# thiery-lab/manifold-mcmc-for-diffusions

Hardware: AMD Instinct MI355X
Metric: constrained-leapfrog steps/sec (all chains), FHN noisy-obs 400 sub-steps (higher is better)
Workload: dtype f64; 1 GPU; FHN noisy-obs, T=100 obs, S=400 steps/obs, R=5 obs/subseq, sigma_y=0.1, 256 chains per GPU (BASELINE.json configs[1]), Newton solver, standard splitting; chains_per_gpu=256, global_chains=256, dim_q=80106, traj_len=16, stepping=chmc_leapfrog_steps per trajectory (batched steps), chain_steps_nominal=152576, parallelism=chains x1 (no data-path collective, 1 gather), ranks_joined=1, collective_world_size=1, collective_route=torch.distributed gather, overlap_halves=-1

## Files before the change

### manifold_mcmc_for_diffusions_amd/context.py

```python
import ctypes as C
import numpy as np
from . import _lib
from ._lib import ChmcConfig, as_c, ptr, iptr, check

MODEL_IDS = {"fhn": 0, "sir": 1, "fhn_nb": 2}
STATUS_NAMES = {0: "ok", 1: "not_converged", 2: "diverged", 3: "non_reversible", -1: "inactive"}


class ChmcContext:
    def __init__(self, model, obs_interval, num_steps_per_obs, num_obs_per_subseq, y_seq, sigma=None,
                 use_gaussian_splitting=False, num_chains=1, device=0):
        L = _lib.lib()
        self.L = L
        y = as_c(np.asarray(y_seq).reshape(-1))
        self._y = y
        cfg = ChmcConfig(
            model=MODEL_IDS[model] if isinstance(model, str) else int(model), num_obs=len(y),
            num_steps_per_obs=int(num_steps_per_obs),
            num_obs_per_subseq=0 if num_obs_per_subseq is None else int(num_obs_per_subseq),
            noisy=2 if isinstance(sigma, str) else int(sigma is not None),
            use_gaussian_splitting=int(bool(use_gaussian_splitting)),
            num_chains=int(num_chains), device=int(device), obs_interval=float(obs_interval),
            sigma=0.0 if sigma is None or isinstance(sigma, str) else float(sigma), y_seq=ptr(y))
        h = C.c_void_p()
# ... 296 lines not shown
                      divergence_tol=1e10, max_iters=50, reverse_check_tol=2e-8):
        dt = as_c(np.broadcast_to(np.asarray(dt, dtype=np.float64), (self.B,)))
        act = None if active is None else np.ascontiguousarray(active, dtype=np.int32)
        status = np.zeros(self.B, dtype=np.int32)
        itf, itb = np.zeros(self.B, dtype=np.int32), np.zeros(self.B, dtype=np.int32)
        rev = np.zeros(self.B)
        check(self.L.chmc_leapfrog_step(self.h, ptr(dt), iptr(act), int(n_inner_step), int(newton), constraint_tol,
                                        position_tol, divergence_tol, int(max_iters), reverse_check_tol, iptr(status),
                                        iptr(itf), iptr(itb), ptr(rev)), "chmc_leapfrog_step")
        return dict(status=status, iters_fwd=itf, iters_bwd=itb, rev_err=rev)

    def leapfrog_steps(self, dt, n_steps, active=None, n_inner_step=1, newton=True, constraint_tol=1e-9, position_tol=1e-8,
                       divergence_tol=1e10, max_iters=50, reverse_check_tol=2e-8):
        dt = as_c(np.broadcast_to(np.asarray(dt, dtype=np.float64), (self.B,)))
        act = None if active is None else np.ascontiguousarray(active, dtype=np.int32)
        per_chain = None if np.isscalar(n_steps) else np.ascontiguousarray(np.broadcast_to(n_steps, (self.B,)), dtype=np.int32)
        n_all = int(n_steps) if per_chain is None else 0
        ndone, status = np.zeros(self.B, dtype=np.int32), np.zeros(self.B, dtype=np.int32)
        itf, itb = np.zeros(self.B, dtype=np.int32), np.zeros(self.B, dtype=np.int32)
        rev = np.zeros(self.B)
        check(self.L.chmc_leapfrog_steps(self.h, ptr(dt), iptr(act), iptr(per_chain), n_all, int(n_inner_step), int(newton),
                                         constraint_tol, position_tol, divergence_tol, int(max_iters), reverse_check_tol,
                                         iptr(ndone), iptr(status), iptr(itf), iptr(itb), ptr(rev)), "chmc_leapfrog_steps")
        return dict(n_done=ndone, status=status, iters_fwd=itf, iters_bwd=itb, rev_err=rev)

    def comm_init(self, id128, rank, world):
        buf = (C.c_char * 128).from_buffer_copy(bytes(id128))
        check(self.L.chmc_comm_init(self.h, buf, int(rank), int(world)), "chmc_comm_init")
        self.comm_world = int(world)

    @staticmethod
    def comm_unique_id():
        buf = (C.c_char * 128)()
        check(_lib.lib().chmc_comm_unique_id(buf), "chmc_comm_unique_id")
        return bytes(buf)

    def gather_samples_device(self, local_dev_ptr, count, gathered_dev_ptr):
        check(self.L.chmc_gather_samples(self.h, C.c_void_p(local_dev_ptr), int(count), C.c_void_p(gathered_dev_ptr)),
              "chmc_gather_samples")

    def comm_info(self):
        wd, rk = C.c_int(0), C.c_int(0)
        check(self.L.chmc_comm_info(self.h, C.byref(wd), C.byref(rk)), "chmc_comm_info")
        return wd.value, rk.value

    def comm_destroy(self):
        check(self.L.chmc_comm_destroy(self.h), "chmc_comm_destroy")

    def diagnostics(self):
        out = (C.c_longlong * 80)()
        check(self.L.chmc_get_diagnostics(self.h, out), "chmc_get_diagnostics")
        v = np.array(out[:], dtype=np.int64)
        return dict(par_scan=v[:64], gram_mfma_launches=int(v[64]), gram_valu_launches=int(v[65]),
                    retract_kernel_launches=int(v[66]), traj_kernel_launches=int(v[67]), extra=v[68:80])

    def counters(self):
        out = (C.c_longlong * 8)()
        check(self.L.chmc_get_counters(self.h, out), "chmc_get_counters")
        keys = ("constr", "jacob_constr_blocks", "lu_jacob_product_blocks", "chol_gram_blocks",
                "grad_log_det_sqrt_gram", "leapfrog_step", "projection_iterations", "_")
        return dict(zip(keys, (int(v) for v in out)))
```

### manifold_mcmc_for_diffusions_amd/csrc/backend_hip.h

```cpp
#pragma once
#include <hip/hip_runtime.h>

static thread_local hipStream_t g_stream = nullptr;
static thread_local hipStream_t g_streams[3] = {nullptr, nullptr, nullptr};
static thread_local int g_device = -1;
static hipError_t g_first_err = hipSuccess;

static inline void note(hipError_t e) {
  if (e != hipSuccess && g_first_err == hipSuccess) g_first_err = e;
}
static int dev_set(int device) {
  hipError_t e = hipSetDevice(device);
  if (e != hipSuccess) {
    g_err = std::string("hipSetDevice: ") + hipGetErrorString(e);
    return -1;
  }
  return 0;
}
static int dev_init(int device) {
  int n = 0;
  hipError_t e = hipGetDeviceCount(&n);
  if (e != hipSuccess || n <= 0) {
    g_err = std::string("no HIP device available (") + hipGetErrorString(e) + ")";
    return -1;
// ... 61 lines not shown
  __syncthreads();
  if (threadIdx.x == 0) {
    const unsigned t = atomicAdd(ticket, 1u);
    if (t == gridDim.x - 1) {
      const int v = atomicAdd(counter, 0);
      *ticket = 0u;
      __hip_atomic_store(host_out, v, __ATOMIC_RELEASE, __HIP_MEMORY_SCOPE_SYSTEM);
    }
  }
}
static void d2d(void* dst, const void* src, size_t bytes) {
  note(hipMemcpyAsync(dst, src, bytes, hipMemcpyDeviceToDevice, g_stream));
}
static const int kStagRing = 16;
static thread_local hipEvent_t g_fork_ev = nullptr, g_join_ev[2], g_stag_ev[2][kStagRing];
static thread_local int g_stag_n[2] = {0, 0};
static thread_local int g_cur_half = -1;
static void streams_init_events() {
  if (g_fork_ev) return;
  note(hipEventCreateWithFlags(&g_fork_ev, hipEventDisableTiming));
  for (int h = 0; h < 2; ++h) {
    note(hipEventCreateWithFlags(&g_join_ev[h], hipEventDisableTiming));
    for (int i = 0; i < kStagRing; ++i) note(hipEventCreateWithFlags(&g_stag_ev[h][i], hipEventDisableTiming));
  }
}
static void use_stream(int half) {
  g_cur_half = half;
  g_stream = g_streams[half + 1];
}
static void streams_fork() {
  streams_init_events();
  note(hipEventRecord(g_fork_ev, g_streams[0]));
  for (int h = 0; h < 2; ++h) note(hipStreamWaitEvent(g_streams[h + 1], g_fork_ev, 0));
  g_stag_n[0] = g_stag_n[1] = 0;
}
static void streams_join() {
  for (int h = 0; h < 2; ++h) {
    note(hipEventRecord(g_join_ev[h], g_streams[h + 1]));
    note(hipStreamWaitEvent(g_streams[0], g_join_ev[h], 0));
  }
  use_stream(-1);
}
static const bool g_no_stagger = false;
static void stagger_wait() {
  if (g_cur_half < 0 || g_no_stagger) return;
  const int o = g_cur_half ^ 1;
  if (g_stag_n[o] > 0) note(hipStreamWaitEvent(g_stream, g_stag_ev[o][(g_stag_n[o] - 1) % kStagRing], 0));
}
static void stagger_record() {
  if (g_cur_half < 0 || g_no_stagger) return;
  const int h = g_cur_half;
  note(hipEventRecord(g_stag_ev[h][g_stag_n[h] % kStagRing], g_stream));
  g_stag_n[h]++;
}
static int dev_sync() {
  note(hipStreamSynchronize(g_stream));
  if (g_first_err != hipSuccess) {
    g_err = std::string("HIP error: ") + hipGetErrorString(g_first_err);
    g_first_err = hipSuccess;
    return -1;
  }
  return 0;
}

template <class F>
__global__ void __launch_bounds__(256) k_run(F f, int n) {
  const int tid = blockIdx.x * blockDim.x + threadIdx.x;
  if (tid < n) f(tid);
}
#include <vector>
struct ProfRec {
  hipEvent_t a, b;
  int cls;
};
static unsigned g_prof_mask = 0;
static int g_prof_stride = 1;
static long long g_prof_seen[16];
static inline bool g_prof_on_for(int cls) {
  if (!((g_prof_mask >> cls) & 1u)) return false;
  return (g_prof_seen[cls]++ % g_prof_stride) == 0;
}
static std::vector<ProfRec> g_prof_pending;
static std::vector<hipEvent_t> g_prof_pool;
static double g_prof_ms[16];
static long long g_prof_n[16];
static hipEvent_t prof_event() {
  if (!g_prof_pool.empty()) {
    hipEvent_t e = g_prof_pool.back();
    g_prof_pool.pop_back();
    return e;
  }
  hipEvent_t e;
  note(hipEventCreate(&e));
  return e;
}
static void prof_drain() {
  if (g_prof_pending.empty()) return;
  for (int i = 0; i < 3; ++i)
    if (g_streams[i]) note(hipStreamSynchronize(g_streams[i]));
  for (auto& r : g_prof_pending) {
    float ms = 0.f;
    note(hipEventElapsedTime(&ms, r.a, r.b));
    g_prof_ms[r.cls] += ms;
    g_prof_n[r.cls] += 1;
    g_prof_pool.push_back(r.a);
    g_prof_pool.push_back(r.b);
// ... 226 lines not shown
```

### manifold_mcmc_for_diffusions_amd/csrc/chmc_api.inc

```
#include <string>
#include <algorithm>
#include <vector>
#include <cstring>
#include <cstdio>
#include <cstdlib>
#include <cmath>
#include <thread>
#include "../../include/chmc.h"

using namespace chmc;

static thread_local std::string g_err;
static int fail(const std::string& m) {
  g_err = m;
  return -1;
}
#include CHMC_BACKEND_HEADER

struct chmc_ctx {
  std::thread::id owner = std::this_thread::get_id();
  chmc_config cfg;
  int model, RMt, part, num_partition, npart_sum;
  Sys sy;
  int K[2], C[2];
  std::vector<BlockDesc> hblk[2];
  BlockDesc* d_blk[2];
  int* d_obs2blk[2];
  int* d_order[2];
  double *d_y, *d_xobs, *d_ham;
  Slots sl;
  Work w;
  int *d_itf, *d_itb, *d_act;
  unsigned long long* d_out = nullptr;
  BlockDesc* d_blk_full = nullptr;
  int* d_order_ident = nullptr;
  bool mom_tangent = false;
  bool snap_tangent = false;
  bool have_state = false;
  double* d_m0 = nullptr;
  double *d_tree_part = nullptr, *d_tree_out = nullptr;
  int* d_tree_mask = nullptr;
  TreeState tree{};
  bool have_tree = false;
  bool rows_fresh = false;
  std::vector<unsigned char> h_out;
  double *d_qbak = nullptr, *d_pbak = nullptr;
  std::vector<void*> allocs;
  long long counters[8];
  long long diag[16] = {0};
  bool par_scan = false;
  int par_waves = 1;
  int row_split_sel[2] = {1, 1};
  int round = 0;
  int halves = 1;
  int hB[2] = {0, 0}, hc0[2] = {0, 0};
  int* d_order_half[2][2] = {{nullptr, nullptr}, {nullptr, nullptr}};
  void* comm = nullptr;
  int comm_rank = 0, comm_world = 1;
  double *d_q0 = nullptr, *d_p0 = nullptr;
  int* d_ncommit = nullptr;
  int last_n_inner = 1;
  int proj_rounds[2] = {0, 0}, proj_stable[2] = {0, 0};
  int *d_nsteps = nullptr, *d_ndone = nullptr;
  int num_cus = 256;
  std::vector<double> last_dt;
  std::vector<int> last_active;
  bool last_active_null = true;
};

template <class T_>
static T_* alloc(chmc_ctx* c, size_t n) {
  T_* p = (T_*)dev_alloc(n * sizeof(T_));
  c->allocs.push_back(p);
  return p;
}

static void build_partition(chmc_ctx* c, int p, int init) {
  const chmc_config& g = c->cfg;
  const int T = g.num_obs, R = g.num_obs_per_subseq, S = g.num_steps_per_obs;
  const int X = c->sy.X, V = c->sy.V, V0 = c->sy.V0;
  std::vector<int> sizes;
  if (R <= 0 || R >= T) {
    sizes.push_back(T);
  } else {
    int num_full = (T - init) / R, num_rem = (T - init) % R;
    int num_middle = num_rem == 0 ? num_full - 1 : num_full;
    int final_ = num_rem == 0 ? R : num_rem;
    sizes.push_back(init);
    for (int i = 0; i < num_middle; ++i) sizes.push_back(R);
    sizes.push_back(final_);
  }
  int obs = 0, row = 0;
  for (size_t b = 0; b < sizes.size(); ++b) {
    BlockDesc B;
    memset(&B, 0, sizeof(B));
    B.obs0 = obs, B.nobs = sizes[b], B.first = b == 0, B.last = b + 1 == sizes.size();
    B.ny = (B.last || g.noisy) ? B.nobs : B.nobs - 1;
    B.nrows = B.ny + (B.last ? 0 : X);
    B.row0 = row;
    B.step0 = obs * S, B.nsteps = B.nobs * S;
    B.col0 = B.first ? 0 : V0 + B.step0 * V;
    B.ncols = B.nsteps * V + (B.first ? V0 : 0);
    row += B.nrows, obs += B.nobs;
    c->hblk[p].push_back(B);
  }
  c->K[p] = (int)sizes.size();
  c->C[p] = row;
}

struct ViewSave {
  Sys sy;
  Slots sl;
  Work w;
  int *d_itf, *d_itb, *d_act;
};
// ... 314 lines not shown
    dev_zero(sl.q[s], sizeof(double) * (B * Q + CHMC_Q_PAD)), dev_zero(sl.p[s], sizeof(double) * B * Q);
    dev_zero(sl.grad[s], sizeof(double) * B * Q);
    dev_zero(sl.Jv[s], sizeof(double) * B * RM * sy.NV);
    sl.PB[s] = sl.LF[s] = nullptr;
#ifdef CHMC_WAVE_KERNELS
    if (compact_family(c->RMt)) {
      sl.PB[s] = alloc<double>(c, B * sy.T * sy.S * sy.X * sy.V);
      sl.LF[s] = alloc<double>(c, B * kmax * sy.NOBS * RM * sy.X);
      dev_zero(sl.PB[s], sizeof(double) * B * sy.T * sy.S * sy.X * sy.V);
      dev_zero(sl.LF[s], sizeof(double) * B * kmax * sy.NOBS * RM * sy.X);
    }
#endif
  }
  c->w.muF = sl.PB[0] ? alloc<double>(c, B * kmax * sy.NOBS * sy.X) : nullptr;
  c->w.muF2 = sl.PB[0] ? alloc<double>(c, B * kmax * sy.NOBS * sy.X) : nullptr;
  c->w.ivl = sl.PB[0] ? alloc<double>(c, B * kmax * sy.NOBS * (2 * sy.X * sy.X + sy.X * sy.Z)) : nullptr;
  c->w.gcq = sl.PB[0] && RM > 8 ? alloc<double>(c, B * kmax * sy.NOBS * (2 * sy.X * sy.X + sy.X * sy.Z)) : nullptr;
  c->w.gbw = sl.PB[0] && RM > 8 ? alloc<double>(c, B * kmax * sy.NOBS * (sy.X + 2 * sy.Z)) : nullptr;
  sl.cur = alloc<int>(c, B);
  dev_zero(sl.cur, sizeof(int) * B);
  Work& w = c->w;
  c->npart_sum = rowsum_groups(sy.Q);
  w.trajw = alloc<double>(c, B * sy.TRJ);
  w.cpad = alloc<double>(c, B * kmax * RM), w.tpad = alloc<double>(c, B * kmax * RM);
  w.lampad = alloc<double>(c, B * kmax * RM);
  w.cpad2 = alloc<double>(c, B * kmax * RM), w.lampad2 = alloc<double>(c, B * kmax * RM);
  w.Ew = alloc<double>(c, B * kmax * RM * U), w.Cb = alloc<double>(c, B * kmax * U * U);
  w.sb = alloc<double>(c, B * kmax * U), w.gup = alloc<double>(c, B * kmax * U);
  w.Dw = alloc<double>(c, B * kmax * RM * RM), w.JuL = alloc<double>(c, B * kmax * RM * U);
  w.JvW = (RM > 8 || gram_mfma()) ? alloc<double>(c, B * RM * sy.NV) : nullptr;
  if (w.JvW) dev_zero(w.JvW, sizeof(double) * B * RM * sy.NV);
  w.zbP = alloc<double>(c, B * kmax * RM * sy.Z), w.gMb = alloc<double>(c, B * kmax * RM * RM);
  w.gzd = alloc<double>(c, B * kmax * RM * sy.Z), w.gWu = alloc<double>(c, B * kmax * RM * U);
  w.gxdt = alloc<double>(c, B * kmax * RM * sy.X);
  w.sdt = alloc<double>(c, B), w.cdt = alloc<double>(c, B);
  dev_zero(w.sdt, sizeof(double) * B), dev_zero(w.cdt, sizeof(double) * B);
  w.mu = alloc<double>(c, B * Q), w.qb = alloc<double>(c, B * Q + CHMC_Q_PAD), w.pb = alloc<double>(c, B * Q);
  dev_zero(w.qb, sizeof(double) * (B * Q + CHMC_Q_PAD));
  w.vin = alloc<double>(c, B * Q);
  w.Xd = alloc<double>(c, B * sy.T * sy.S * RM * sy.X);
  w.err = alloc<double>(c, B), w.dt = alloc<double>(c, B);
  c->d_out = alloc<unsigned long long>(c, B + (3 * B * sizeof(int) + 7) / 8);
  w.ndq = alloc<unsigned long long>(c, B), w.rev = c->d_out;
  w.part = alloc<double>(c, B * c->npart_sum * 2);
  w.iters = alloc<int>(c, B), w.nw = alloc<int>(c, B), w.ok = alloc<int>(c, B);
  w.status = reinterpret_cast<int*>(c->d_out + B), w.nstat = alloc<int>(c, B), w.n_active = alloc<int>(c, 12);
  {
    double* z = alloc<double>(c, 256);
    dev_zero(z, sizeof(double) * 256);
    w.zeros = z;
  }
  w.ticket = alloc<unsigned>(c, B);
  dev_zero(w.ticket, sizeof(unsigned) * B);
  w.nfallback = alloc<int>(c, 128);
  dev_zero(w.nfallback, sizeof(int) * 128);
  c->d_itf = w.status + B, c->d_itb = w.status + 2 * B, c->d_act = alloc<int>(c, B);
  c->d_ham = alloc<double>(c, B * 4);
  dev_zero(w.cpad, sizeof(double) * B * kmax * RM);
  dev_zero(w.lampad, sizeof(double) * B * kmax * RM);
  dev_zero(w.cpad2, sizeof(double) * B * kmax * RM), dev_zero(w.lampad2, sizeof(double) * B * kmax * RM);
  dev_zero(w.dt, sizeof(double) * B);
  select_partition(c, 0);
  if (dev_sync()) {
    std::string e = g_err;
    chmc_destroy(c);
    return fail("chmc_create: " + e);
  }
  *out = c;
  return 0;
}

extern "C" int chmc_comm_destroy(chmc_ctx* ctx);
extern "C" void chmc_destroy(chmc_ctx* c) {
  if (!c) return;
  if (c->comm) chmc_comm_destroy(c);
  for (void* p : c->allocs) dev_free(p);
  delete c;
}

extern "C" int chmc_get_dims(const chmc_ctx* c, int* d) {
  if (!c || !d) return fail("chmc_get_dims: null argument");
  const Sys& s = c->sy;
  int v[16] = {s.B, s.Q, s.NV, s.U, s.X, s.T, s.S, c->num_partition, s.RM, s.Kmax,
               c->C[0], c->num_partition > 1 ? c->C[1] : 0, c->K[0], c->num_partition > 1 ? c->K[1] : 0, s.V, s.V0};
  memcpy(d, v, sizeof(v));
  return 0;
}
extern "C" int chmc_get_blocks(const chmc_ctx* c, int p, int* out) {
  if (!c || !out || p < 0 || p >= c->num_partition) return fail("chmc_get_blocks: bad argument");
  memcpy(out, c->hblk[p].data(), sizeof(BlockDesc) * c->K[p]);
  return 0;
}
extern "C" int chmc_get_counters(const chmc_ctx* c, long long* out8) {
  if (!c || !out8) return fail("chmc_get_counters: null argument");
  memcpy(out8, c->counters, sizeof(c->counters));
  return 0;
}

static void begin_all(chmc_ctx* c, const double* d_dt, const int* d_active, double dt_scale = 1.0) {
  launch(KBegin{c->w, d_active, d_dt, dt_scale}, c->sy.B);
}

static bool lean16(const chmc_ctx* c) {
  return c->sy.RM > 8 && compact16(c) && row_split_for(c) > 1;
}
static bool chain16(const chmc_ctx* c) { return chain16_layout(c->sy.Kmax, c->sy.RM) && compact16(c) && lean16(c); }
// ... 249 lines not shown
          if (c->sl.PB[0]) {
            launch_blocks(k_newton_ivl<M>, (long)sy.B * sy.K * sy.NOBS, 64, 1, sy, c->sl, c->w, prev, qsel);
            launch_blocks(k_newton_comb<M, RM>, (long)sy.B * sy.K, 64, 1, sy, c->sl, c->w, prev, qsel);
          } else if (gram_mfma8(c)) {
            launch_wave(k_rev_wave<M, RM, 1, false>, (long)sy.B * sy.K, 1, sy, c->sl, c->w, prev, qsel);
            launch_blocks(k_gram_rows_mfma<RM>, (long)sy.B * sy.K, 64, 1, sy, c->sl, c->w, prev, 1, qsel), c->diag[0]++;
          } else {
            launch_wave(k_rev_wave<M, RM, 1>, (long)sy.B * sy.K, 1, sy, c->sl, c->w, prev, qsel);
          }
        }
      }
      if constexpr (RM > 8) {
        if (!fused16)
          launch_blocks(k_newton_factor_wave<M, RM>, ((long)sy.B * sy.K + 3) / 4, 64, 9, sy, c->sl, c->w, prev, qsel);
      } else if (fused) {
        launch_blocks(k_newton_fsm_wave<M, RM>, (long)sy.B, 64, 5, sy, c->sl, c->w, prev, qsel);
      } else {
        launch(KNewtonFactor<M, RM>{sy, c->sl, c->w, prev}, (long)sy.B * sy.K, 9);
      }
#else
      launch(KNewtonBlk<M, RM>{sy, c->sl, c->w, prev, qsel}, (long)sy.B * sy.K, 1);
#endif
      if (!fused && !fused16) CHMC_SOLVE_CHAIN(M, RM, 0, 0, sy, c->sl, c->w, prev, qsel, 0);
    } else {
      launch(KSymBlk<M, RM>{sy, c->sl, c->w, prev, 1}, (long)sy.B * sy.K, 9);
      CHMC_SOLVE_CHAIN(M, RM, 1, 0, sy, c->sl, c->w, prev, qsel, 0);
    }
#ifdef CHMC_WAVE_KERNELS
    if (RM <= 8 ? c->sl.PB[0] != nullptr : compact16(c)) {
      if (!fused && !fused16) launch(KMuF<RM, M::X, 0>{sy, c->sl, c->w, prev}, (long)sy.B * sy.K * sy.NOBS * M::X, 5);
      launch_colmax(KUpdatePB<RM, M::X, M::V, 0, 1>{sy, c->sl, c->w, prev, qsel, 0, chk ? *chk : CheckArgs{}},
                    sy.T * sy.S + sy.V0 + (sy.noisy ? sy.T : 0), sy.B, 4);
    } else
#endif
    CHMC_UPDATE(0, sy, c->sl, c->w, prev, qsel, 0);
  });
}

static int retract_waves(const chmc_ctx* c, int newton, const void* views) {
#ifdef CHMC_WAVE_KERNELS
  const char* e = getenv("CHMC_RETRACT_KERNEL");
  int want = e ? atoi(e) : (c->sy.B <= c->num_cus ? 1 : (c->sy.B <= CHMC_CHAIN_WG4_MAX_PER_CU * c->num_cus ? 2 : 0));
  if (!(newton && !views && c->sy.K == 1 && c->sy.RM > 8 && compact16(c))) want = 0;
  return want == 1 ? CHMC_RETRACT_WAVES : want == 2 ? 4 : 0;
#else
  (void)c, (void)newton, (void)views;
  return 0;
#endif
}
static bool retract_kernel(const chmc_ctx* c, int newton, const void* views) { return retract_waves(c, newton, views) != 0; }
static bool traj_kernel(const chmc_ctx* c, int n_inner, int newton) {
  return retract_kernel(c, newton, nullptr) && lean16(c) && n_inner == 1 && c->mom_tangent && c->halves == 1;
}
static int run_projection(chmc_ctx* c, int newton, int prev, int qsel, double ctol, double ptol, double dtol,
                          int max_iters, const ViewSave* views = nullptr, int count_dir = -1) {
  const Sys& sy = c->sy;
#ifdef CHMC_WAVE_KERNELS
  if (retract_kernel(c, newton, views)) {
    int* iters_dst = count_dir < 0 ? nullptr : (count_dir ? c->d_itb : c->d_itf);
    CHMC_DISPATCH(c, {
      if constexpr (RM == 16) {
        if (retract_waves(c, newton, views) == 4)
          launch_blocks(k_retract_chain<M, RM, 4>, (long)sy.B, 256, 1, sy, c->sl, c->w, prev, qsel, ctol, ptol, dtol, max_iters,
                        iters_dst);
        else
          launch_blocks(k_retract_chain<M, RM, CHMC_RETRACT_WAVES>, (long)sy.B, 64 * CHMC_RETRACT_WAVES, 1, sy, c->sl, c->w, prev,
                        qsel, ctol, ptol, dtol, max_iters, iters_dst);
      }
    });
    c->counters[6]++;
    c->diag[2]++;
    return 0;
  }
#endif
  const int nh = views ? 2 : 1;
  auto enter = [&](int h) {
    if (views) set_half(c, *views, h);
  };
  for (int h = 0; h < nh; ++h) {
    enter(h);
    if (sy.B > 0) launch(KNewtonBegin{c->w}, sy.B);
  }
  int fwd_guess = 2;
#ifdef CHMC_WAVE_KERNELS
  const bool carry = c->par_scan && sy.K == 1;
#else
  const bool carry = false;
#endif
  const int max_rounds = carry ? 12 * (max_iters + 1) : max_iters;
  const bool fused_check = update_fuses_check(c);
  auto iteration = [&](int poll_slot) {
    iteration_scan(c, newton, prev, qsel, fwd_guess, 1);
    if (fused_check) {
      dev_zero(c->w.n_active, sizeof(int));
      const CheckArgs chk{ctol, ptol, dtol, max_iters, 1, count_dir < 0 ? nullptr : (count_dir ? c->d_itb : c->d_itf)};
      iteration_after_scan(c, newton, prev, qsel, &chk);
    } else {
      iteration_after_scan(c, newton, prev, qsel);
      const KCheck chk{c->w, ctol, ptol, dtol, max_iters, sy.B, count_dir < 0 ? nullptr : (count_dir ? c->d_itb : c->d_itf),
                       c->round & 3};
      if (poll_slot >= 0) launch_publish(chk, sy.B, c->w.n_active + (c->round & 3), poll_slot);
      else launch(chk, sy.B);
      return;
    }
    if (poll_slot >= 0) poll_begin(poll_slot, c->w.n_active + (c->round & 3));
  };
  bool done[2] = {false, nh == 1};
  for (int h = 0; h < nh; ++h) {
    enter(h);
    if (sy.B <= 0) done[h] = true;
  }
  int& expect = c->proj_rounds[prev & 1];
  int& stable = c->proj_stable[prev & 1];
  const bool predict = !views && stable >= 3 && expect >= 2;
  int rounds_done = 0;
  for (int it = 0; it < max_rounds && !(done[0] && done[1]); ++it) {
    if (predict && it >= expect && poll_end((it - 1) & 1) == 0) {
      done[0] = true;
      break;
    }
    for (int h = 0; h < nh; ++h) {
      if (done[h]) continue;
      enter(h);
      fwd_guess = it == 0 ? 2 : 1;
      c->round = it;
      iteration(it >= 1 ? 2 * h + (it & 1) : -1);
    }
    c->counters[6]++;
    if (it == 0) continue;
    bool all_empty = true;
    for (int h = 0; h < nh; ++h) {
      if (done[h]) continue;
      if (it >= 2 && poll_end(2 * h + ((it - 1) & 1)) == 0) {
        done[h] = true;
        continue;
      }
      all_empty = false;
      if (it + 1 >= max_rounds) poll_end(2 * h + (it & 1));
    }
    if (all_empty) c->counters[6]--;
    else rounds_done = it + 1;
  }
  if (!views) {
    if (predict && done[0] && rounds_done < expect) rounds_done = expect;
    stable = rounds_done == expect ? stable + 1 : 0;
    expect = rounds_done;
  }
  for (int h = 0; h < nh; ++h) {
    enter(h);
    if (sy.B > 0) launch(KNewtonEnd{c->w, count_dir < 0 ? nullptr : (count_dir ? c->d_itb : c->d_itf)}, sy.B);
  }
  c->round = 0;
  return 0;
}

static int check_ctx(const chmc_ctx* c, const char* fn) {
  if (!c) return fail(std::string(fn) + ": null context");
  if (c->owner != std::this_thread::get_id())
    return fail(std::string(fn) + ": a context must be driven by the host thread that created it");
  return 0;
}
#define CHMC_ENTER(fn)                 \
  if (check_ctx(ctx, fn)) return -1;   \
  use_stream(-1);                      \
  if (dev_set(ctx->cfg.device)) return fail(std::string(fn) + ": " + g_err);
#define CHMC_LEAVE(fn)                                                 \
  if (dev_sync()) return fail(std::string(fn) + ": " + g_err);        \
  return 0;

extern "C" int chmc_get_diagnostics(chmc_ctx* ctx, long long* out80) {
  CHMC_ENTER("chmc_get_diagnostics")
  if (!out80) return fail("chmc_get_diagnostics: null output");
  int ps[80];
  d2h(ps, ctx->w.nfallback, sizeof(ps));
  for (int i = 0; i < 64; ++i) out80[i] = ps[i];
  for (int i = 0; i < 16; ++i) out80[64 + i] = ctx->diag[i];
#ifdef CHMC_RETRACT_PROF
  for (int i = 4; i < 16; ++i) out80[64 + i] = ps[64 + i - 4];
#endif
  CHMC_LEAVE("chmc_get_diagnostics")
}

extern "C" int chmc_set_state(chmc_ctx* ctx, const double* q, const double* p, const double* x_obs, int partition) {
  CHMC_ENTER("chmc_set_state")
  if (!q || !x_obs) return fail("chmc_set_state: q and x_obs_seq are required");
  if (partition < 0 || partition >= ctx->num_partition) return fail("chmc_set_state: partition out of range");
// ... 696 lines not shown
    dev_zero(ctx->d_itf, sizeof(int) * sy.B), dev_zero(ctx->d_itb, sizeof(int) * sy.B);
    CHMC_DISPATCH(ctx, {
      if constexpr (RM == 16) {
        if (retract_waves(ctx, newton, nullptr) == 4)
          launch_blocks(k_traj_chain<M, RM, 4>, (long)sy.B, 256, 1, sy, ctx->sl, ctx->w,
                        n_steps_host ? ctx->d_nsteps : nullptr, n_steps_all, ctol, ptol, dtol, max_iters, rev_tol, ctx->d_itf,
                        ctx->d_itb, want_n_done ? ctx->d_ndone : nullptr);
        else
          launch_blocks(k_traj_chain<M, RM, CHMC_RETRACT_WAVES>, (long)sy.B, 64 * CHMC_RETRACT_WAVES, 1, sy, ctx->sl, ctx->w,
                        n_steps_host ? ctx->d_nsteps : nullptr, n_steps_all, ctol, ptol, dtol, max_iters, rev_tol, ctx->d_itf,
                        ctx->d_itb, want_n_done ? ctx->d_ndone : nullptr);
      }
    });
    ctx->rows_fresh = false;
    ctx->diag[3]++;
    const int ns = n_steps_host ? 1 : n_steps_all;
    ctx->counters[0] += ns, ctx->counters[1] += ns, ctx->counters[3] += ns, ctx->counters[4] += ns, ctx->counters[6] += 2 * ns;
    return 0;
  }
#endif
  const bool two = ctx->halves == 2;
  const ViewSave full = save_view(ctx);
  const int nh = two ? 2 : 1;
  const double kick = 0.5 * n_inner;
  auto enter = [&](int h) {
    if (two) set_half(ctx, full, h);
    return (size_t)(two ? ctx->hc0[h] : 0);
  };
  if (two) streams_fork();
  for (int h = 0; h < nh; ++h) {
    const size_t c0 = enter(h);
    begin_all(ctx, d_dt ? ctx->w.err : nullptr, d_active ? ctx->d_act : nullptr, 1.0 / n_inner);
    dev_zero(ctx->d_itf, sizeof(int) * sy.B), dev_zero(ctx->d_itb, sizeof(int) * sy.B);
    if (n_inner > 1) {
      dev_zero(ctx->d_ncommit + c0, sizeof(int) * sy.B);
      launch(KGatherState{sy, ctx->sl, ctx->d_q0 + c0 * sy.Q, ctx->d_p0 + c0 * sy.Q}, (long)sy.B * sy.Q, 8);
    }
  }
  for (int i = 0; i < n_inner; ++i) {
    const bool last = i == n_inner - 1;
    for (int h = 0; h < nh; ++h) {
      enter(h);
      if (i > 0) {
        launch_rows(KFlow{sy, ctx->sl, ctx->w, 0, 0, 0, 1.0}, sy.Q, sy.B, 8);
      } else if (ctx->mom_tangent) {
        if (pending_kick) launch_rows(KKick2FlowPg{sy, ctx->sl, ctx->w, kick}, sy.Q, sy.B, 8);
        else launch_rows(KKickFlowPg{sy, ctx->sl, ctx->w, kick}, sy.Q, sy.B, 8);
      } else {
        launch(KKick{sy, ctx->sl, ctx->w, 0, 1, kick}, (long)sy.B * sy.Q, 8);
        project_momentum(ctx, 0, 3, 2);
        launch_rows(KFlow{sy, ctx->sl, ctx->w, 0, 0, 1, 1.0}, sy.Q, sy.B, 8);
      }
    }
    run_projection(ctx, newton, 0, 0, ctol, ptol, dtol, max_iters, two ? &full : nullptr, 0);
    for (int h = 0; h < nh; ++h) {
      enter(h);
      state_eval_core(ctx, 1, last, 3);
      const bool fix_in_jw = last && mom_fix_in_jw(ctx);
      if (fix_in_jw)
        launch_rows(KMomFixEdges{KMomFixInitPg{sy, ctx->sl, ctx->w, 1}}, sy.U + sy.V0 + (sy.Q - sy.U - sy.NV), sy.B, 8);
      else
        launch_rows(KMomFixInitPg{sy, ctx->sl, ctx->w, 1}, sy.Q, sy.B, 8);
      const bool flow_in_update = last && rev_flow_in_update(ctx);
      if (last)
        project_momentum_and_kick_direction(ctx, 1, false, fix_in_jw, flow_in_update);
      else
        project_momentum(ctx, 1, 0, 0);
      launch_rows(KFlow{sy, ctx->sl, ctx->w, 1, 1, 0, -1.0}, flow_in_update ? sy.U : sy.Q, sy.B, 8);
    }
    run_projection(ctx, newton, 1, 1, ctol, ptol, dtol, max_iters, two ? &full : nullptr, 1);
    for (int h = 0; h < nh; ++h) {
      const size_t c0 = enter(h);
      launch_colmax(KRevDiff{sy, ctx->sl, ctx->w}, (sy.Q + 1) / 2, sy.B, 8);
      launch(KRevCheck{ctx->w, rev_tol}, sy.B);
      if (last) {
        if (!skip_end_kick) launch_rows(KKickPg{sy, ctx->sl, ctx->w, 1, 0, kick}, sy.Q, sy.B, 8);
        launch(KCommit{ctx->sl, ctx->w}, sy.B);
      } else {
        launch(KCommitInner{ctx->sl, ctx->w, ctx->d_ncommit + c0}, sy.B);
      }
    }
  }
  if (two) {
    restore_view(ctx, full);
    streams_join();
    const int extra = n_inner;
    ctx->counters[0] -= extra, ctx->counters[1] -= extra, ctx->counters[3] -= extra, ctx->counters[4] -= 1;
  }
  return 0;
}
static void step_finish(chmc_ctx* ctx, bool masked, int n_inner, int* status, int* iters_fwd, int* iters_bwd,
                        double* rev_err) {
  const Sys& sy = ctx->sy;
  bool any_failed = false;
  {
    const size_t nb = (size_t)sy.B * (sizeof(double) + 3 * sizeof(int));
    ctx->h_out.resize(nb);
    d2h(ctx->h_out.data(), ctx->d_out, nb);
    const unsigned char* h = ctx->h_out.data();
    if (rev_err) memcpy(rev_err, h, sizeof(double) * sy.B);
    h += sizeof(double) * sy.B;
    if (status) memcpy(status, h, sizeof(int) * sy.B);
    if (iters_fwd) memcpy(iters_fwd, h + sizeof(int) * sy.B, sizeof(int) * sy.B);
    if (iters_bwd) memcpy(iters_bwd, h + 2 * sizeof(int) * sy.B, sizeof(int) * sy.B);
    const int* st = reinterpret_cast<const int*>(h);
    for (int c = 0; c < sy.B; ++c) any_failed = any_failed || st[c] > 0;
    if (n_inner > 1 && any_failed) {
      std::vector<int> nc(sy.B), mask(sy.B);
      d2h(nc.data(), ctx->d_ncommit, sizeof(int) * sy.B);
      bool any = false;
      for (int c = 0; c < sy.B; ++c) any = (mask[c] = st[c] > 0 && nc[c] > 0) || any;
      if (any) {
        h2d(ctx->d_act, mask.data(), sizeof(int) * sy.B);
        ctx->last_active_null = true;
        ctx->last_active.clear();
        launch(KInnerRestore{sy, ctx->sl, ctx->d_q0, ctx->d_p0, ctx->d_act}, (long)sy.B * sy.Q, 8);
        launch(KBegin{ctx->w, ctx->d_act, nullptr, 1.0}, sy.B);
        state_eval(ctx, 0);
        h2d(ctx->w.status, st, sizeof(int) * sy.B);
      }
    }
  }
  ctx->counters[5]++;
  ctx->mom_tangent = ctx->mom_tangent || (!masked && !any_failed);
}
extern "C" int chmc_leapfrog_step(chmc_ctx* ctx, const double* dt, const int* active, int n_inner, int newton,
                                  double ctol, double ptol, double dtol, int max_iters, double rev_tol, int* status,
                                  int* iters_fwd, int* iters_bwd, double* rev_err) {
  CHMC_ENTER("chmc_leapfrog_step")
  if (!dt) return fail("chmc_leapfrog_step: dt is required");
  if (n_inner < 1) return fail("chmc_leapfrog_step: n_inner_step must be at least 1");
  if (step_enqueue(ctx, dt, active, nullptr, n_inner, newton, ctol, ptol, dtol, max_iters, rev_tol)) return -1;
  step_finish(ctx, active != nullptr, n_inner, status, iters_fwd, iters_bwd, rev_err);
  CHMC_LEAVE("chmc_leapfrog_step")
// ... 324 lines not shown
```

### manifold_mcmc_for_diffusions_amd/csrc/chmc_core.h

```cpp
#pragma once
#include <math.h>
#include <stdint.h>
#include "chmc_model.h"

#define CHMC_FI __attribute__((always_inline))
#if defined(__HIPCC__)
#define CHMC_UNROLL _Pragma("unroll")
#define CHMC_UNROLL4 _Pragma("unroll 4")
#else
#define CHMC_UNROLL
#define CHMC_UNROLL4
#endif

namespace chmc {

#ifndef CHMC_FWD_DEPTH
#define CHMC_FWD_DEPTH 4
#endif
#define CHMC_Q_PAD 256
#define CHMC_TPAD 16

struct BlockDesc {
  int obs0, nobs, first, last;
  int row0, nrows, ny;
// ... 1741 lines not shown
struct KCheck {
  Work w;
  double ctol, ptol, dtol;
  int max_iters, B;
  int* iters_dst;
  int slot;
  CHMC_HD void operator()(int c) const {
    if (c == 0) w.n_active[(slot + 1) & 3] = 0;
    if (!w.nw[c]) return;
    if (w.nw[c] != 1) {
      atomic_add_i32(w.n_active + slot, 1);
      return;
    }
    const int i = ++w.iters[c];
    const double err = w.err[c], ndq = bitsd(w.ndq[c]);
    const bool diverged = (err > dtol) || (err != err);
    const bool converged = (err < ctol) && (ndq < ptol);
    if (i >= max_iters || diverged || converged) {
      w.nw[c] = 0;
      int st = converged ? 0 : (diverged ? 2 : 1);
      w.nstat[c] = st;
      if (st) w.ok[c] = 0, w.status[c] = st;
      if (iters_dst) iters_dst[c] += i;
    } else {
      atomic_add_i32(w.n_active + slot, 1);
    }
  }
};

struct KNewtonBegin {
  Work w;
  CHMC_HD void operator()(int c) const {
    w.nw[c] = w.ok[c];
    w.iters[c] = 0;
    w.err[c] = -1.0;
    w.ndq[c] = 0x7ff0000000000000ULL;
    w.nstat[c] = 0;
    if (c == 0) w.n_active[0] = 0;
  }
};

struct KNewtonEnd {
  Work w;
  int* iters_dst;
  CHMC_HD void operator()(int c) const {
    if (!w.nw[c]) return;
    w.nw[c] = 0;
    w.nstat[c] = 1;
    w.ok[c] = 0, w.status[c] = 1;
    if (iters_dst) iters_dst[c] += w.iters[c];
  }
};

template <int RM>
struct KJw {
  Sys sy;
  Slots sl;
  Work w;
  int which, vsel_;
  CHMC_HD void operator()(int tid) const {
    const int i = tid % RM;
    const int cbk = tid / RM;
    const int c = cbk / sy.K;
    const int b = cbk - c * sy.K;
    if (!w.ok[c]) return;
    const BlockDesc bd = sy.blk[b];
    const int s = sl.cur[c] ^ which;
    const bool minv = (vsel_ & 256) != 0;
    const int vsel = vsel_ & 255;
    const double* vct = (vsel == 0 ? pick(sl.p, s) : vsel == 1 ? w.pb : vsel == 2 ? w.vin : vsel == 4 ? pick(sl.pg, s) : pick(sl.p, s ^ 1)) + (size_t)c * sy.Q;
    const size_t cb = (size_t)c * sy.Kmax + b;
    double acc = 0.0;
    if (i < bd.nrows) {
      const double* ju = pick(sl.JuP, s) + (cb * RM + i) * sy.U;
      for (int a = 0; a < sy.U; ++a) acc += ju[a] * (minv ? metric_inv_u(sy, vct, a) : vct[a]);
      const double* Jv = pick(sl.Jv, s) + ((size_t)c * RM + i) * sy.NV + bd.col0;
      const double* wv = vct + sy.U + bd.col0;
      double a2 = 0.0;
      for (int k = 0; k < bd.ncols; ++k) a2 += Jv[k] * wv[k];
      acc += a2;
      if (sy.noisy && i < bd.ny) acc += sigma_at(sy, pick(sl.q, s) + (size_t)c * sy.Q) * vct[sy.U + sy.NV + bd.obs0 + i];
    }
    w.cpad[cb * RM + i] = acc;
  }
};

struct KKick {
  Sys sy;
  Slots sl;
  Work w;
  int which, out_other;
  double hfrac;
  CHMC_HD void operator()(int tid) const {
    const int c = tid / sy.Q;
    if (!w.ok[c]) return;
    const int s = sl.cur[c] ^ which;
    const double h = hfrac * w.dt[c];
    const double g = pick(sl.grad, s)[tid] + (sy.gaussian ? 0.0 : pick(sl.q, s)[tid]);
    const double pin = pick(sl.p, s)[tid];
    (out_other ? pick(sl.p, s ^ 1) : pick(sl.p, s))[tid] = pin - h * g;
  }
};
struct KInitPg {
  Sys sy;
  Slots sl;
  Work w;
// ... 635 lines not shown
```

Before: 51980 steps/s.

## Offload Newton projection tail chains to a side stream overlapping next phase

When only a small fraction of chains (at most a quarter) remain unconverged in the Newton projection loop, those chains are split off into a separate work mask and their remaining iterations run on a side HIP stream. Meanwhile the converged chains proceed through the following momentum/flow or reversibility-check phase on the main stream, and the phase is then replayed for the tail chains before their mask is merged back. The goal is to cut the serial latency of many nearly empty projection rounds. In exchange it adds extra phase launches, event syncs, host polling and complexity around counter bookkeeping.

```diff
diff --git a/manifold_mcmc_for_diffusions_amd/context.py b/manifold_mcmc_for_diffusions_amd/context.py
--- a/manifold_mcmc_for_diffusions_amd/context.py
+++ b/manifold_mcmc_for_diffusions_amd/context.py
@@ -372,7 +372,8 @@
         check(self.L.chmc_get_diagnostics(self.h, out), "chmc_get_diagnostics")
         v = np.array(out[:], dtype=np.int64)
         return dict(par_scan=v[:64], gram_mfma_launches=int(v[64]), gram_valu_launches=int(v[65]),
-                    retract_kernel_launches=int(v[66]), traj_kernel_launches=int(v[67]), extra=v[68:80])
+                    retract_kernel_launches=int(v[66]), traj_kernel_launches=int(v[67]), tail_splits=int(v[68]),
+                    tail_chain_rounds=int(v[69]), extra=v[68:80])
 
     def counters(self):
         out = (C.c_longlong * 8)()
diff --git a/manifold_mcmc_for_diffusions_amd/csrc/backend_hip.h b/manifold_mcmc_for_diffusions_amd/csrc/backend_hip.h
--- a/manifold_mcmc_for_diffusions_amd/csrc/backend_hip.h
+++ b/manifold_mcmc_for_diffusions_amd/csrc/backend_hip.h
@@ -137,6 +137,22 @@
   const int h = g_cur_half;
   note(hipEventRecord(g_stag_ev[h][g_stag_n[h] % kStagRing], g_stream));
   g_stag_n[h]++;
+}
+#define CHMC_BACKEND_TAIL_STREAM 1
+static thread_local hipEvent_t g_tail_ev[4] = {nullptr, nullptr, nullptr, nullptr};
+static void use_side_stream(bool on) {
+  g_cur_half = -1;
+  g_stream = g_streams[on ? 1 : 0];
+}
+static void tail_fork(int dir) {
+  if (!g_tail_ev[0])
+    for (int i = 0; i < 4; ++i) note(hipEventCreateWithFlags(&g_tail_ev[i], hipEventDisableTiming));
+  note(hipEventRecord(g_tail_ev[2 * dir], g_streams[0]));
+  note(hipStreamWaitEvent(g_streams[1], g_tail_ev[2 * dir], 0));
+}
+static void tail_join(int dir) {
+  note(hipEventRecord(g_tail_ev[2 * dir + 1], g_streams[1]));
+  note(hipStreamWaitEvent(g_streams[0], g_tail_ev[2 * dir + 1], 0));
 }
 static int dev_sync() {
   note(hipStreamSynchronize(g_stream));
diff --git a/manifold_mcmc_for_diffusions_amd/csrc/chmc_api.inc b/manifold_mcmc_for_diffusions_amd/csrc/chmc_api.inc
--- a/manifold_mcmc_for_diffusions_amd/csrc/chmc_api.inc
+++ b/manifold_mcmc_for_diffusions_amd/csrc/chmc_api.inc
@@ -16,6 +16,11 @@
   return -1;
 }
 #include CHMC_BACKEND_HEADER
+#ifndef CHMC_BACKEND_TAIL_STREAM
+static void use_side_stream(bool) {}
+static void tail_fork(int) {}
+static void tail_join(int) {}
+#endif
 
 struct chmc_ctx {
   std::thread::id owner = std::this_thread::get_id();
@@ -61,6 +66,16 @@
   int* d_ncommit = nullptr;
   int last_n_inner = 1;
   int proj_rounds[2] = {0, 0}, proj_stable[2] = {0, 0};
+  struct TailRun {
+    bool pending = false;
+    int it0 = 0;
+    int newton = 0, prev = 0, qsel = 0, max_iters = 0, count_dir = -1;
+    double ctol = 0.0, ptol = 0.0, dtol = 0.0;
+  } tail;
+  bool tail_allowed = false;
+  int *d_tail_ok = nullptr, *d_tail_nw = nullptr;
+  Work w_main;
+  int n_after[2][16];
   int *d_nsteps = nullptr, *d_ndone = nullptr;
   int num_cus = 256;
   std::vector<double> last_dt;
@@ -481,6 +496,10 @@
   }
   w.ticket = alloc<unsigned>(c, B);
   dev_zero(w.ticket, sizeof(unsigned) * B);
+  c->d_tail_ok = alloc<int>(c, B), c->d_tail_nw = alloc<int>(c, B);
+  dev_zero(c->d_tail_ok, sizeof(int) * B), dev_zero(c->d_tail_nw, sizeof(int) * B);
+  for (int d = 0; d < 2; ++d)
+    for (int r = 0; r < 16; ++r) c->n_after[d][r] = -1;
   w.nfallback = alloc<int>(c, 128);
   dev_zero(w.nfallback, sizeof(int) * 128);
   c->d_itf = w.status + B, c->d_itb = w.status + 2 * B, c->d_act = alloc<int>(c, B);
@@ -836,6 +855,55 @@
 static bool traj_kernel(const chmc_ctx* c, int n_inner, int newton) {
   return retract_kernel(c, newton, nullptr) && lean16(c) && n_inner == 1 && c->mom_tangent && c->halves == 1;
 }
+static bool tail_stream_applies(const chmc_ctx* c) {
+  const char* e = getenv("CHMC_TAIL_STREAM");
+  if (e && atoi(e) == 0) return false;
+  return c->halves == 1 && !c->par_scan && c->sy.Kmax > 1 && c->model != CHMC_MODEL_SIR;
+}
+static int tail_threshold(const chmc_ctx* c) { return c->sy.B >= 4 ? c->sy.B / 4 : 1; }
+static void tail_enter(chmc_ctx* c) {
+  c->w_main = c->w;
+  c->w.ok = c->d_tail_ok, c->w.nw = c->d_tail_nw, c->w.n_active = c->w_main.n_active + 4;
+  use_side_stream(true);
+}
+static void tail_leave(chmc_ctx* c) {
+  c->w = c->w_main;
+  use_side_stream(false);
+}
+static int tail_run_projection(chmc_ctx* c) {
+  chmc_ctx::TailRun& t = c->tail;
+  const Sys& sy = c->sy;
+  t.pending = false;
+  const int dir = t.prev & 1;
+  int n = poll_end((t.it0 - 1) & 1);
+  if (t.it0 - 1 < 16) c->n_after[dir][t.it0 - 1] = n;
+  const int n_tail = n;
+  int rounds_done = t.it0;
+  if (n_tail > 0) {
+    int* iters_dst = t.count_dir < 0 ? nullptr : (t.count_dir ? c->d_itb : c->d_itf);
+    tail_enter(c);
+    c->diag[4]++;
+    for (int it = t.it0; it < t.max_iters && n > 0; ++it) {
+      c->round = it;
+      iteration_scan(c, t.newton, t.prev, t.qsel, 1, 1);
+      iteration_after_scan(c, t.newton, t.prev, t.qsel, nullptr);
+      const KCheck chk{c->w, t.ctol, t.ptol, t.dtol, t.max_iters, sy.B, iters_dst, it & 3};
+      launch_publish(chk, sy.B, c->w.n_active + (it & 3), 2 + (it & 1));
+      c->counters[6]++;
+      c->diag[5] += n;
+      rounds_done = it + 1;
+      n = poll_end(2 + (it & 1));
+      if (it < 16) c->n_after[dir][it] = n;
+    }
+    launch(KNewtonEnd{c->w, iters_dst}, sy.B);
+    c->round = 0;
+  }
+  int& expect = c->proj_rounds[dir];
+  int& stable = c->proj_stable[dir];
+  stable = rounds_done == expect ? stable + 1 : 0;
+  expect = rounds_done;
+  return n_tail;
+}
 static int run_projection(chmc_ctx* c, int newton, int prev, int qsel, double ctol, double ptol, double dtol,
                           int max_iters, const ViewSave* views = nullptr, int count_dir = -1) {
   const Sys& sy = c->sy;
@@ -898,10 +966,29 @@
   int& stable = c->proj_stable[prev & 1];
   const bool predict = !views && stable >= 3 && expect >= 2;
   int rounds_done = 0;
+  const bool tail_ok = c->tail_allowed && !views && !carry && !fused_check;
+  const int dir = prev & 1;
+  int n_seen = -1;
   for (int it = 0; it < max_rounds && !(done[0] && done[1]); ++it) {
-    if (predict && it >= expect && poll_end((it - 1) & 1) == 0) {
-      done[0] = true;
-      break;
+    if (predict && it >= expect) {
+      n_seen = poll_end((it - 1) & 1);
+      if (n_seen == 0) {
+        done[0] = true;
+        break;
+      }
+    }
+    if (tail_ok && it >= 2) {
+      const int thr = tail_threshold(c);
+      const int last = it - 1 < 16 ? c->n_after[dir][it - 1] : -1;
+      if ((predict && it == expect - 1 && last > 0 && last <= thr) || (n_seen > 0 && n_seen <= thr)) {
+        launch(KTailSplit{c->w, c->d_tail_ok, c->d_tail_nw, c->w.n_active + 4, it & 3}, sy.B);
+        tail_fork(dir);
+        c->tail.pending = true, c->tail.it0 = it;
+        c->tail.newton = newton, c->tail.prev = prev, c->tail.qsel = qsel, c->tail.max_iters = max_iters;
+        c->tail.count_dir = count_dir, c->tail.ctol = ctol, c->tail.ptol = ptol, c->tail.dtol = dtol;
+        c->round = 0;
+        return 0;
+      }
     }
     for (int h = 0; h < nh; ++h) {
       if (done[h]) continue;
@@ -915,7 +1002,12 @@
     bool all_empty = true;
     for (int h = 0; h < nh; ++h) {
       if (done[h]) continue;
-      if (it >= 2 && poll_end(2 * h + ((it - 1) & 1)) == 0) {
+      const int left = it >= 2 ? poll_end(2 * h + ((it - 1) & 1)) : -1;
+      if (!views && it >= 2) {
+        n_seen = left;
+        if (it - 1 < 16) c->n_after[dir][it - 1] = left;
+      }
+      if (it >= 2 && left == 0) {
         done[h] = true;
         continue;
       }
@@ -1718,7 +1810,21 @@
         launch_rows(KFlow{sy, ctx->sl, ctx->w, 0, 0, 1, 1.0}, sy.Q, sy.B, 8);
       }
     }
+    auto with_tail = [&](int dir, auto&& phases) {
+      phases();
+      if (!ctx->tail.pending) return;
+      if (tail_run_projection(ctx) > 0) {
+        long long keep[4] = {ctx->counters[0], ctx->counters[1], ctx->counters[3], ctx->counters[4]};
+        phases();
+        ctx->counters[0] = keep[0], ctx->counters[1] = keep[1], ctx->counters[3] = keep[2], ctx->counters[4] = keep[3];
+        tail_leave(ctx);
+        tail_join(dir);
+        launch(KTailMerge{ctx->w, ctx->d_tail_ok}, sy.B);
+      }
+    };
+    ctx->tail_allowed = !two && tail_stream_applies(ctx);
     run_projection(ctx, newton, 0, 0, ctol, ptol, dtol, max_iters, two ? &full : nullptr, 0);
+    with_tail(0, [&] {
     for (int h = 0; h < nh; ++h) {
       enter(h);
       state_eval_core(ctx, 1, last, 3);
@@ -1734,7 +1840,9 @@
         project_momentum(ctx, 1, 0, 0);
       launch_rows(KFlow{sy, ctx->sl, ctx->w, 1, 1, 0, -1.0}, flow_in_update ? sy.U : sy.Q, sy.B, 8);
     }
+    });
     run_projection(ctx, newton, 1, 1, ctol, ptol, dtol, max_iters, two ? &full : nullptr, 1);
+    with_tail(1, [&] {
     for (int h = 0; h < nh; ++h) {
       const size_t c0 = enter(h);
       launch_colmax(KRevDiff{sy, ctx->sl, ctx->w}, (sy.Q + 1) / 2, sy.B, 8);
@@ -1746,6 +1854,8 @@
         launch(KCommitInner{ctx->sl, ctx->w, ctx->d_ncommit + c0}, sy.B);
       }
     }
+    });
+    ctx->tail_allowed = false;
   }
   if (two) {
     restore_view(ctx, full);
diff --git a/manifold_mcmc_for_diffusions_amd/csrc/chmc_core.h b/manifold_mcmc_for_diffusions_amd/csrc/chmc_core.h
--- a/manifold_mcmc_for_diffusions_amd/csrc/chmc_core.h
+++ b/manifold_mcmc_for_diffusions_amd/csrc/chmc_core.h
@@ -1817,6 +1817,26 @@
   }
 };
 
+struct KTailSplit {
+  Work w;
+  int *ok_t, *nw_t, *n_active_t;
+  int slot;
+  CHMC_HD void operator()(int c) const {
+    const int t = w.nw[c] == 1;
+    nw_t[c] = t;
+    ok_t[c] = t ? w.ok[c] : 0;
+    if (t) w.nw[c] = 0, w.ok[c] = 0;
+    if (c == 0) n_active_t[slot] = 0;
+  }
+};
+struct KTailMerge {
+  Work w;
+  const int* ok_t;
+  CHMC_HD void operator()(int c) const {
+    if (ok_t[c]) w.ok[c] = 1;
+  }
+};
+
 template <int RM>
 struct KJw {
   Sys sy;
```

New measurement: 51480 steps/s. No clear change (-1.0%).
